# spaceandtimefdn/blitzar

Hardware: AMD Instinct MI355X
Metric: MSM throughput (scalar-point ops/sec) (higher is better)
Workload: dtype u32; 1 GPU; curve25519_msm_n2^20_252bit; columns_per_gpu=1, rows=1048576, parallelism=columns x1

## Files before the change

### __graft_entry__.py

```python
import os
import subprocess
import sys

ROOT = os.path.dirname(os.path.abspath(__file__))
if ROOT not in sys.path:
    sys.path.insert(0, ROOT)


def build():
    from blitzar_amd import build as bz_build
    bz_build.build()
    hooks_dir = os.path.join(ROOT, "tests", "native", "_build")
    os.makedirs(hooks_dir, exist_ok=True)
    hooks = os.path.join(hooks_dir, "libbz_hooks.so")
    src = os.path.join(ROOT, "tests", "native", "hooks.cpp")
    if not os.path.exists(hooks) or os.path.getmtime(hooks) < os.path.getmtime(src):
        subprocess.run(["g++", "-O2", "-std=c++20", "-fPIC", "-shared", "-I" + ROOT, src, "-o", hooks],
                       check=True)
    src = os.path.join(ROOT, "tests", "native", "tile_digest_check.cc")
    newest = max(os.path.getmtime(src),
                 os.path.getmtime(os.path.join(ROOT, "blitzar_amd", "csrc", "msm", "tile_digest.h")))
    for exe, flags in (("tile_digest_check", ["-O2"]),
                       ("tile_digest_check_san", ["-O1", "-g", "-fsanitize=address,undefined",
                                                  "-fno-sanitize-recover=all"])):
        exe = os.path.join(hooks_dir, exe)
        if not os.path.exists(exe) or os.path.getmtime(exe) < newest:
            subprocess.run(["g++", *flags, "-std=c++20", "-I" + ROOT, src, "-o", exe], check=True)
    src = os.path.join(ROOT, "tests", "native", "batch_normalise_check.cc")
    newest = os.path.getmtime(src)
    for d, _, fs in os.walk(os.path.join(ROOT, "blitzar_amd", "csrc")):
        newest = max([newest] + [os.path.getmtime(os.path.join(d, f)) for f in fs if f.endswith(".h")])
    for exe, flags in (("batch_normalise_check", ["-O2"]),
                       ("batch_normalise_check_san", ["-O1", "-g", "-fsanitize=address,undefined",
                                                      "-fno-sanitize-recover=all"])):
        exe = os.path.join(hooks_dir, exe)
        if not os.path.exists(exe) or os.path.getmtime(exe) < newest:
            subprocess.run(["g++", *flags, "-std=c++20", "-I" + ROOT, src, "-o", exe], check=True)
    pb_dir = os.path.join(ROOT, "tools", "pipeline_bench")
    lib_so = os.path.join(ROOT, "blitzar_amd", "lib", "libblitzar_amd.so")
    os.makedirs(os.path.join(pb_dir, "_build"), exist_ok=True)
    for tool in ("pipeline_bench", "multi_device_check", "hostapi_bench", "caller_table_bench"):
        exe = os.path.join(pb_dir, "_build", tool)
        src = os.path.join(pb_dir, tool + ".cc")
        if (not os.path.exists(exe)
                or os.path.getmtime(exe) < max(os.path.getmtime(src), os.path.getmtime(lib_so))):
            subprocess.run(["/opt/rocm/bin/hipcc", "-O2", "-std=c++17",
                            "-I" + os.path.join(ROOT, "include"), "-I" + pb_dir, src,
                            "-L" + os.path.dirname(lib_so), "-lblitzar_amd",
                            "-Wl,-rpath,$ORIGIN/../../../blitzar_amd/lib", "-o", exe], check=True)
    mc_src = os.path.join(ROOT, "tools", "multi_commitment", "benchmark.cc")
    mc_exe = os.path.join(ROOT, "tools", "multi_commitment", "_build", "multi_commitment")
    os.makedirs(os.path.dirname(mc_exe), exist_ok=True)
    if (not os.path.exists(mc_exe)
            or os.path.getmtime(mc_exe) < max(os.path.getmtime(mc_src), os.path.getmtime(lib_so))):
        subprocess.run(["g++", "-O2", "-std=c++17", "-I" + os.path.join(ROOT, "include"), mc_src,
                        "-L" + os.path.dirname(lib_so), "-lblitzar_amd",
                        "-Wl,-rpath,$ORIGIN/../../../blitzar_amd/lib", "-Wl,-rpath,/opt/rocm/lib",
                        "-o", mc_exe], check=True)
    exe = os.path.join(hooks_dir, "sig_ours")
    src = os.path.join(ROOT, "tests", "native", "boundary", "signatures.cc")
    if (not os.path.exists(exe)
            or os.path.getmtime(exe) < max(os.path.getmtime(src), os.path.getmtime(lib_so))):
        subprocess.run(["g++", "-O1", "-std=c++17", "-I" + os.path.join(ROOT, "include"),
                        '-DBZ_API_HEADER="blitzar_api.h"', src, "-L" + os.path.dirname(lib_so),
                        "-lblitzar_amd", "-Wl,-rpath,$ORIGIN/../../../blitzar_amd/lib",
                        "-Wl,-rpath,/opt/rocm/lib", "-o", exe], check=True)
    mt_dir = os.path.join(ROOT, "tools", "mt19937")
    mt_so = os.path.join(mt_dir, "_build", "libmtstream.so")
    mt_src = os.path.join(mt_dir, "mtstream.cc")
    os.makedirs(os.path.dirname(mt_so), exist_ok=True)
    if not os.path.exists(mt_so) or os.path.getmtime(mt_so) < os.path.getmtime(mt_src):
        subprocess.run(["g++", "-O2", "-std=c++17", "-fPIC", "-shared", "-pthread", mt_src, "-o",
                        mt_so], check=True)
    subprocess.run([sys.executable, os.path.join(ROOT, "oracle", "ref", "build_ref.py")], check=True)
    from tests import device_hooks
    device_hooks.build()
    import blitzar_amd.api as api
    api.load()


def smoke():
    import numpy as np
    from blitzar_amd import api
    from oracle import ref_oracle
    lib = api.load()
    assert lib.bzamd_device_count() > 0, "smoke() needs a GPU"
    api.reset_for_testing()
    assert api.init(api.SXT_GPU_BACKEND, 16) == 0
    rng = np.random.default_rng(0)
    n = 1000
    cols = [(rng.integers(0, 256, (n, 32), dtype=np.uint8), False),
            (rng.integers(0, 256, (n, 4), dtype=np.uint8), True)]
    before = lib.bzamd_kernel_launch_count()
    got = api.compute_pedersen_commitments(0, cols)
    assert lib.bzamd_kernel_launch_count() > before, "no kernels were launched"
    if ref_oracle.available():
        want = ref_oracle.commit(0, cols, ref_oracle.ristretto_generators(n))
        assert np.array_equal(got, want), "HIP MSM disagrees with the reference oracle"
    golden = api.compute_pedersen_commitments(0, [(np.array([2000, 7500, 5000, 1500], np.uint32), False)])
    assert golden[0, :4].tolist() == [4, 105, 58, 131]
    a = rng.integers(0, 256, (5, 32), dtype=np.uint8)
    b = rng.integers(0, 256, (5, 32), dtype=np.uint8)
    t0 = api.transcript_new("smoke")
    l, r, ap, t1 = api.prove_inner_product(t0, 5, 2, a, b)
    if ref_oracle.available():
        wl, wr, wap, wt = ref_oracle.ip_prove(t0, 5, 2, a, b)
        assert np.array_equal(l, wl) and np.array_equal(r, wr) and np.array_equal(ap, wap)
        assert np.array_equal(t1, wt), "inner-product proof disagrees with the reference prover"
    api.reset_for_testing()
    print("smoke ok")


if __name__ == "__main__":
    build()
```

### blitzar_amd/csrc/msm/curve_traits.h

```cpp
#pragma once

#include "blitzar_amd/csrc/curve/ed25519.h"
#include "blitzar_amd/csrc/curve/ed29.h"
#include "blitzar_amd/csrc/curve/ed16_wave.h"
#include "blitzar_amd/csrc/curve/sw29.h"
#include "blitzar_amd/csrc/curve/sw29_coop.h"
#include "blitzar_amd/csrc/curve/sw_wave.h"
#include "blitzar_amd/csrc/curve/weierstrass.h"

namespace bz {

template <int N> struct sw_api_affine {
  u64 X[N];
  u64 Y[N];
  u8 infinity;
};
static_assert(sizeof(sw_api_affine<4>) == 72);
static_assert(sizeof(sw_api_affine<6>) == 104);

struct ed25519_msm {
  static constexpr unsigned curve_id = 0;
  using point = ed29_point;
  using addend = ed29_cached_packed;
  using api_projective = ed_point;
// ... 3 lines not shown
  static constexpr size_t output_size = 32;
  static constexpr size_t projective_size = 160;
  static constexpr int accumulate_waves_per_simd = 3;
  static constexpr int accumulate_launch_waves = 2;
  static constexpr bool has_batched_prepare = false;
  static constexpr double call_table_entry_cost = 1.0;

  BZ_HD static point identity() { return ed29::identity(); }
  BZ_HD static point add(const point& a, const point& b) { return ed29::add(a, b); }
  BZ_HD static point dbl_n(const point& a, int k) { return ed29::dbl_n(a, k); }
  BZ_HD static point neg(const point& a) { return ed29::neg(a); }
  BZ_HD static void accumulate(point& acc, const addend& q, bool negate) {
    acc = ed29::add_cached(acc, ed29::unpack(q), negate);
  }
  using operand = ed29_cached;
  BZ_HD static operand stage(const addend& q) {
    operand o = ed29::unpack(q);
    f29::pin(o.YpX);
    f29::pin(o.YmX);
    f29::pin(o.Z);
    f29::pin(o.T2d);
    return o;
  }
  BZ_HD static void accumulate(point& acc, const operand& q, bool negate) {
    acc = ed29::add_cached(acc, q, negate);
  }
  static constexpr bool has_signed_gather = true;
  BZ_HD static addend gather(const addend* table, u32 row, bool negate) {
    return ed29::gather_signed(table, row, negate);
  }
  BZ_HD static void accumulate_gathered(point& acc, const operand& q, bool negate) {
    acc = ed29::add_cached_presigned(acc, q, negate);
  }
  static constexpr bool first_pinned = true;
  BZ_HD static point first_gathered(const operand& q, bool negate) {
    return ed29::from_cached_presigned(q, negate);
  }
  BZ_HD static addend make_addend(const void* api_generators, u64 i) {
    return ed29::pack(ed29::cached_from_ed(static_cast<const ed_point*>(api_generators)[i]));
  }
  BZ_HD static addend addend_from_api_projective(const void* projective, u64 i) {
    return make_addend(projective, i);
  }
  BZ_HD static void encode(u8* out, const point& p) { ristretto29::encode(out, p); }
  BZ_HD static void store_projective(u8* out, const point& p) {
    *reinterpret_cast<ed_point*>(out) = ed29::to_ed(p);
  }
  BZ_HD static point point_from_api_projective(const void* projective, u64 i) {
    return ed29::from_ed(static_cast<const ed_point*>(projective)[i]);
  }
  BZ_HD static void store_api_generator(u8* out, const point& p) { store_projective(out, p); }
  BZ_HD static point point_from_api_generator(const void* api_generators, u64 i) {
    return point_from_api_projective(api_generators, i);
  }
  static constexpr u32 batch_points_per_lane = 4;
  using batch_fe = fe29;
  BZ_HD static fe29 batch_one() { return f29::one(); }
  BZ_HD static fe29 batch_mul(const fe29& a, const fe29& b) { return f29::mul(a, b); }
  BZ_HD static bool batch_is_zero(const fe29& a) { return f29::is_zero(a); }
  BZ_HD static fe29 batch_z(const point& p, bool& is_identity) {
    is_identity = false;
    return p.Z;
  }
  static constexpr size_t compact_size = 120;
  BZ_HD static void store_compact(u8* out, const point& p, const fe29& zinv, bool) {
    const fe29 x = f29::mul(p.X, zinv), y = f29::mul(p.Y, zinv);
    const fe51 c[3] = {f29::to_fe51(x), f29::to_fe51(y), f29::to_fe51(f29::mul(x, y))};
    u64* o = reinterpret_cast<u64*>(out);
    for (int k = 0; k < 3; ++k)
      for (int i = 0; i < 5; ++i) o[5 * k + i] = c[k].v[i];
  }
#if defined(__HIPCC__)
  __device__ static fe29 batch_wave_invert(const fe29& z) {
    return batch_wave_invert(z, ed16w::wave_scratch());
  }
  __device__ static fe29 batch_wave_invert(const fe29& z, ed16w::scratch* lds) {
    const ed16w::lane_ctx c = ed16w::make_ctx(lds);
    const fe29 t = ed16w::pow22523(c, z);
    return f29::mul(f29::sqn(t, 3), f29::mul(f29::sq(z), z));
  }
#endif
  static constexpr bool has_wave_horner = true;
#if defined(__HIPCC__)
  __device__ static point wave_horner(const point& acc, bool have_acc, point* window_sums,
                                      u32 stride, u32 num_windows, u32 window_bits) {
    const ed16w::lane_ctx c = ed16w::make_ctx(ed16w::wave_scratch());
    for (u32 w = c.lane; w < num_windows; w += 64) {
      point* slot = window_sums + static_cast<size_t>(w) * stride;
      const ed29_cached_packed q = ed29::pack(ed29::to_cached(*slot));
      *reinterpret_cast<ed29_cached_packed*>(slot) = q;
    }
    ed16w::wave_lds_sync();
    u32 state = ed16w::identity(c);
    if (have_acc) state = ed16w::load_point(c, acc);
    for (u32 i = num_windows; i-- > 0;) {
      if (have_acc || i + 1 != num_windows) {
        for (u32 k = 0; k < window_bits; ++k) state = ed16w::dbl(c, state);
      }
      const u32* q = reinterpret_cast<const u32*>(window_sums + static_cast<size_t>(i) * stride);
      state = ed16w::add_cached(c, state, ed16w::load_words(c, q));
    }
    return ed16w::store_point(c, state);
  }
  __device__ static void wave_chain(point* out, u64 stride, const point& g, u32 windows, u32 bits) {
    const ed16w::lane_ctx c = ed16w::make_ctx(ed16w::wave_scratch());
    u32 state = ed16w::load_point(c, g);
#pragma unroll 1
    for (u32 w = 0;; ++w) {
      const point p = ed16w::store_point(c, state);
      if (c.lane == 0) out[static_cast<u64>(w) * stride] = p;
      if (w + 1 >= windows) break;
#pragma unroll 1
      for (u32 k = 0; k < bits; ++k) state = ed16w::dbl(c, state);
    }
  }
  static constexpr bool has_wave_add_multiple = true;
  static constexpr bool reduce_scan_few_columns_only = false;
  __device__ static point wave_add_multiple(const point& v, const point& s, u32 m) {
    __shared__ ed29_cached_packed addend[2];
    const ed16w::lane_ctx c = ed16w::make_ctx(ed16w::wave_scratch());
    if (c.lane < 2) addend[c.lane] = ed29::pack(ed29::to_cached(c.lane == 0 ? s : v));
    ed16w::wave_lds_sync();
    const u32 sq = ed16w::load_words(c, addend[0].w), vq = ed16w::load_words(c, addend[1].w);
    u32 state = ed16w::identity(c);
    for (int bit = 31 - __builtin_clz(m); bit >= 0; --bit) {
      state = ed16w::dbl(c, state);
      if ((m >> bit) & 1) state = ed16w::add_cached(c, state, sq);
    }
    state = ed16w::add_cached(c, state, vq);
    return ed16w::store_point(c, state);
  }
  static constexpr bool has_wave_encode = true;
  static constexpr bool has_coop_add = false;
  __device__ static void wave_encode(u8* out, const point& p) {
    const ed16w::lane_ctx c = ed16w::make_ctx(ed16w::wave_scratch());
    u64 w[4];
    ristretto29::encode_words(w, p, [&c](const fe29& z) { return ed16w::pow22523(c, z); });
    if (c.lane == 0) {
      for (int i = 0; i < 4; ++i)
        for (int j = 0; j < 8; ++j) out[8 * i + j] = static_cast<u8>(w[i] >> (8 * j));
    }
  }
#endif
};

struct ed25519_niels_msm : ed25519_msm {
  using addend = ed29_niels;
  static constexpr int accumulate_launch_waves = accumulate_waves_per_simd;
  BZ_HD static void accumulate(point& acc, const addend& q, bool negate) {
    acc = ed29::add_niels(acc, q, negate);
  }
  BZ_HD static point first(const addend& q, bool negate) { return ed29::from_niels(q, negate); }
  static constexpr bool has_signed_gather = false;
  static constexpr double call_table_entry_cost = 0.88;
  using operand = ed29_niels;
  BZ_HD static operand stage(const addend& q) {
    operand o = q;
    f29::pin(o.YpX);
    f29::pin(o.YmX);
    f29::pin(o.T2d);
    return o;
  }
  BZ_HD static addend make_addend(const void* api_generators, u64 i) {
    return ed29::to_niels(ed29::from_ed(static_cast<const ed_point*>(api_generators)[i]));
  }
  BZ_HD static addend addend_from_api_projective(const void* projective, u64 i) {
    return make_addend(projective, i);
  }
  static constexpr bool has_batched_prepare = true;
  BZ_HD static fe29 batch_load_z(const void* api_generators, u64 i) {
    return f29::from_fe51(static_cast<const ed_point*>(api_generators)[i].Z);
  }
  BZ_HD static void batch_load_xyz(const void* api_generators, u64 i, fe29& big_x, fe29& big_y,
                                   fe29& z) {
    const ed_point& g = static_cast<const ed_point*>(api_generators)[i];
    big_x = f29::from_fe51(g.X);
    big_y = f29::from_fe51(g.Y);
    z = f29::from_fe51(g.Z);
  }
#if defined(__HIPCC__)
  using batch_scratch = ed16w::scratch;
#endif
  BZ_HD static addend batch_make_addend(const void* api_generators, u64 i, const fe29& zinv) {
    const ed_point& g = static_cast<const ed_point*>(api_generators)[i];
    return niels_of(f29::from_fe51(g.X), f29::from_fe51(g.Y), zinv);
  }
  BZ_HD static addend addend_from_point(const point& p, const fe29& zinv, bool) {
    return niels_of(p.X, p.Y, zinv);
  }
  BZ_HD static addend niels_of(const fe29& big_x, const fe29& big_y, const fe29& zinv) {
    const fe29 x = f29::mul(big_x, zinv);
    const fe29 y = f29::mul(big_y, zinv);
    ed29_niels n;
    n.YpX = f29::weak_reduce(f29::add(y, x));
    n.YmX = f29::weak_reduce(f29::sub(y, x));
    n.T2d = f29::mul(f29::mul(x, y), f29::const_2d());
    for (int k = 0; k < 5; ++k) n.pad[k] = 0;
    return n;
  }
};

template <class G29, unsigned CurveId> struct sw_msm_base {
  static constexpr unsigned curve_id = CurveId;
  static constexpr double call_table_entry_cost = 1.0;
  using G64 = typename G29::G64;
  using F64 = typename G64::F;
  static constexpr int N64 = F64::N;
  using point = typename G29::point;
  using addend = typename G29::packed;
  using api_projective = typename G64::point;
  using api_affine = sw_api_affine<N64>;
  static constexpr size_t api_generator_size = sizeof(api_affine);
  static constexpr size_t projective_size = sizeof(api_projective);
  static constexpr int accumulate_waves_per_simd = G29::N <= 9 ? 3 : 2;
  static constexpr int accumulate_launch_waves = accumulate_waves_per_simd;
  static constexpr bool accumulate_pinned = G29::N <= 9;
  static constexpr bool has_batched_prepare = false;
  static constexpr bool has_signed_gather = false;
  static constexpr bool has_wave_encode = false;
  static constexpr bool has_wave_add_multiple = true;
  static constexpr bool reduce_scan_few_columns_only = true;
#if defined(__HIPCC__)
  __device__ static point wave_add_multiple(const point& v, const point& s, u32 m) {
    using W = sww::wave<G29>;
    const typename W::ctx c = W::make_ctx(sww::wave_scratch());
    const u32 sq = W::load_point_value(c, s), vq = W::load_point_value(c, v);
    u32 st = sq;
    for (int bit = 30 - __builtin_clz(m); bit >= 0; --bit) {
      st = W::dbl(c, st);
      if ((m >> bit) & 1) st = W::add(c, st, sq);
    }
    return W::store_point(c, W::add(c, st, vq));
  }
#endif
  static constexpr bool has_wave_horner = true;
#if defined(__HIPCC__)
  __device__ static void wave_chain(point* out, u64 stride, const point& g, u32 windows, u32 bits) {
    using W = sww::wave<G29>;
    const typename W::ctx c = W::make_ctx(sww::wave_scratch());
    u32 st = W::load_point_value(c, g);
#pragma unroll 1
    for (u32 w = 0;; ++w) {
      const point p = W::store_point(c, st);
      if (c.lane == 0) out[static_cast<u64>(w) * stride] = p;
      if (w + 1 >= windows) break;
#pragma unroll 1
      for (u32 k = 0; k < bits; ++k) st = W::dbl(c, st);
    }
  }
  __device__ static point wave_horner(point acc, bool have_acc, point* window_sums,
                                      u32 stride, u32 num_windows, u32 window_bits) {
    return sww::wave<G29>::horner(sww::wave_scratch(), acc, have_acc, window_sums, stride,
                                  num_windows, window_bits);
  }
#endif

  static constexpr bool has_coop_add = true;
#if defined(__HIPCC__)
  __device__ static point add_coop4(const point& a, const point& b, u32 role) {
    return sw29_coop::add_coop4<G29>(a, b, role);
  }
#endif

  using F29 = typename G29::F;
  using batch_fe = typename G29::fe;
  BZ_HD static batch_fe batch_one() { return F29::one(); }
  BZ_HD static batch_fe batch_mul(const batch_fe& a, const batch_fe& b) { return F29::mul(a, b); }
  BZ_HD static batch_fe batch_z(const point& p, bool& is_identity) {
    is_identity = F29::is_zero(p.Z);
    return is_identity ? F29::one() : p.Z;
  }
  BZ_HD static batch_fe batch_wave_invert(const batch_fe& z) { return F29::invert(z); }
  static constexpr size_t compact_size = 16 * N64;
  BZ_HD static void store_compact(u8* out, const point& p, const batch_fe& zinv, bool is_identity) {
    u64* o = reinterpret_cast<u64*>(out);
    if (is_identity) {
      const typename G64::F::fe one = G64::F::one();
      for (int k = 0; k < N64; ++k) {
        o[k] = k == N64 - 1 ? ~u64{0} : 0;
        o[N64 + k] = one.v[k];
      }
      return;
    }
    F29::to_mont64(o, F29::mul(p.X, zinv));
    F29::to_mont64(o + N64, F29::mul(p.Y, zinv));
  }

  BZ_HD static point identity() { return G29::identity(); }
  BZ_HD static point add(const point& a, const point& b) { return G29::add(a, b); }
  BZ_HD static point dbl_n(const point& a, int k) { return G29::dbl_n(a, k); }
  BZ_HD static void accumulate(point& acc, const addend& q, bool negate) {
    if (G29::is_identity_addend(q)) return;
    acc = G29::template add_mixed<accumulate_pinned>(acc, G29::unpack(q), negate);
  }
  struct operand {
    typename G29::affine a;
    u32 nonzero;
  };
  BZ_HD static operand stage(const addend& q) {
    u64 any = 0;
#pragma unroll
    for (int i = 0; i < N64; ++i) any |= q.x[i] | q.y[i];
    operand o{G29::unpack(q), static_cast<u32>(any) | static_cast<u32>(any >> 32)};
    F29::pin(o.a.x);
    F29::pin(o.a.y);
#if defined(__HIP_DEVICE_COMPILE__)
// ... 78 lines not shown
```

### blitzar_amd/csrc/msm/kernels.h

```cpp
#pragma once

#include <utility>

#include "blitzar_amd/csrc/msm/batch_tree.h"
#include "blitzar_amd/csrc/msm/curve_traits.h"
#include "blitzar_amd/csrc/msm/plan.h"
#include "blitzar_amd/csrc/msm/recode.h"
#include "blitzar_amd/csrc/msm/tile_digest.h"

namespace bz {

using i16 = int16_t;
using i32 = int32_t;
template <class D> inline constexpr u32 kDigitsPerVector = 16 / sizeof(D);

constexpr u32 kSortThreads = 1024;
constexpr u32 kReduceHeavyHeads = 16;
constexpr u32 kReduceMaxHeavy = 8;
constexpr u32 kAccumulateThreads = 256;
constexpr u32 kCombineThreads = 256;

template <class C>
__global__ void __launch_bounds__(256)
    k_prepare_addends(typename C::addend* __restrict__ addends, const void* __restrict__ api_generators,
                      u64 n) {
  const u64 i = static_cast<u64>(blockIdx.x) * blockDim.x + threadIdx.x;
  if (i >= n) return;
  addends[i] = C::make_addend(api_generators, i);
}

template <class C, u32 T>
__device__ __forceinline__ void tree_products(typename C::batch_fe* tree, u32 tid) {
  __syncthreads();
  for (u32 s = T / 2; s >= 1; s >>= 1) {
    tree_product_step<C>(tree, s, tid);
    __syncthreads();
  }
}
template <class C, u32 T>
__device__ __forceinline__ void tree_inverses(typename C::batch_fe* tree, u32 tid) {
  __syncthreads();
  for (u32 s = 1; s < T; s <<= 1) {
    tree_inverse_step<C>(tree, s, tid);
    __syncthreads();
  }
}

__device__ __forceinline__ void wave_lds_fence() {
  __builtin_amdgcn_fence(__ATOMIC_RELEASE, "workgroup");
  __builtin_amdgcn_wave_barrier();
  __builtin_amdgcn_fence(__ATOMIC_ACQUIRE, "workgroup");
}
struct caller_table_view {
  tile_digest* tiles;
  tile_digest* rows;
  u64 valid_rows;
  unsigned long long* converted;
};
constexpr u32 kConvertedCounters = 256, kConvertedCounterStride = 16;
template <class C, bool Table = false>
__global__ void __launch_bounds__(256)
    k_prepare_addends_staged(typename C::addend* __restrict__ addends,
                             const void* __restrict__ api_generators, u64 n,
                             caller_table_view table) {
  using addend = typename C::addend;
  constexpr bool Norm = Table && C::has_batched_prepare;
  static_assert(Table || !C::has_batched_prepare, "Z = 1 addends outside a table: the batched kernel");
  constexpr u32 G = static_cast<u32>(C::api_generator_size);
  constexpr u32 A = static_cast<u32>(sizeof(addend));
  static_assert(G % 8 == 0 && A % 16 == 0 && A <= G && (64 * G) % 16 == 0);
  __shared__ __attribute__((aligned(16))) u8 stage[4 * 64 * G];
  const u32 lane = threadIdx.x & 63;
  const u32 wave = Table ? __builtin_amdgcn_readfirstlane(threadIdx.x >> 6) : threadIdx.x >> 6;
  const u64 first = (static_cast<u64>(blockIdx.x) * 4 + wave) * 64;
  if constexpr (!Norm) {
    if (first >= n) return;
  }
  const u32 count = first >= n ? 0 : static_cast<u32>(n - first < 64 ? n - first : 64);
  bool convert = count != 0;
  u8* region = stage + wave * (64 * G);
  const u8* src = static_cast<const u8*>(api_generators) + first * G;
  const u32 in_bytes = count * G;
  const u64 tile = first >> 6;
  tile_digest state{}, stored{};
  bool tile_known = false;
  if constexpr (Table) {
    tile_known = convert && first < table.valid_rows;
    if (tile_known) stored = table.tiles[tile];
    state = digest_lane_begin(lane, count);
  }
  constexpr u32 kRounds = (64 * G / 16 + 63) / 64;
  uint4 words[kRounds];
#pragma unroll
  for (u32 r = 0; r < kRounds; ++r) {
    const u32 off = (r * 64 + lane) * 16;
    if (off + 16 <= in_bytes) words[r] = *reinterpret_cast<const uint4*>(src + off);
  }
#pragma unroll
  for (u32 r = 0; r < kRounds; ++r) {
    const u32 off = (r * 64 + lane) * 16;
    if (off + 16 <= in_bytes) {
      const uint4 v = words[r];
      *reinterpret_cast<uint4*>(region + off) = v;
      if constexpr (Table) {
        state = digest_absorb(state, off >> 4, v.x | static_cast<u64>(v.y) << 32,
                              v.z | static_cast<u64>(v.w) << 32);
      }
    }
  }
  if ((in_bytes & 8) != 0 && lane == 0) {
    const u64 v = *reinterpret_cast<const u64*>(src + in_bytes - 8);
    *reinterpret_cast<u64*>(region + in_bytes - 8) = v;
    if constexpr (Table) state = digest_absorb(state, in_bytes >> 4, v, 0);
  }
  tile_digest whole{}, mine{};
  if constexpr (Table) {
    state = digest_lane_end(state);
    for (int m = 32; m >= 1; m >>= 1) {
      state.a ^= __shfl_xor(state.a, m, 64);
      state.b ^= __shfl_xor(state.b, m, 64);
    }
    whole = digest_finish(state, count);
    if (tile_known && stored.a == whole.a && stored.b == whole.b) {
      if constexpr (!Norm) return;
      convert = false;
    }
  }
  if (convert) wave_lds_fence();
  if (Table && convert) {
    const bool known = lane < count && first + lane < table.valid_rows;
    tile_digest was{};
    if (known) was = table.rows[first + lane];
    bool same = lane >= count;
    if (lane < count) {
      mine = digest_of_row(reinterpret_cast<const u64*>(region + lane * G), G, lane);
      same = known && was.a == mine.a && was.b == mine.b;
    }
    if (__all(same)) {
      if (count == 64 && lane == 0) table.tiles[tile] = whole;
      if constexpr (!Norm) return;
      convert = false;
    }
  }
  addend a;
  if constexpr (Norm) {
    using fe = typename C::batch_fe;
    constexpr u32 T = 256;
    static_assert(sizeof(fe) * 2 * T % 16 == 0 &&
                  sizeof(fe) * 2 * T + sizeof(typename C::batch_scratch) <= sizeof(stage));
    const bool live = convert && lane < count;
    fe big_x, big_y, z;
    if (live) C::batch_load_xyz(region, lane, big_x, big_y, z);
    wave_lds_fence();
    if (lane == 0) *reinterpret_cast<u32*>(region) = convert ? 1u : 0u;
    __syncthreads();
    u32 any = 0;
#pragma unroll
    for (u32 w = 0; w < 4; ++w) any |= *reinterpret_cast<const u32*>(stage + w * (64 * G));
// ... 854 lines not shown
        run_base[b0 + 1] = gstart1 + (c1 != 0 ? atomicAdd(&fill[b0 + 1], c1) : 0);
      }
      lds_barrier();
#pragma unroll
      for (u32 k = 0; k < kLocalSortPerThread; ++k) {
        const bool active = tid + k * kGroupSortThreads < total;
        const u32 b = (mine[k] >> shift) & in_group;
        const u32 pos = wave_aggregated_add(cursor, b, active);
        if (active) staging[pos] = mine[k];
      }
      lds_barrier();
      u32* out = sorted + task.entry_base + group_begin;
      u32* seg = segment_bucket + task.segment_base;
      const u32 seg_log2 = task.segment_log2, seg_mask = (1u << seg_log2) - 1;
      for (u32 i = tid; i < total; i += kGroupSortThreads) {
        const u32 r = staging[i];
        const u32 b = (r >> shift) & in_group;
        const u32 at = run_base[b] + (i - local_start[b]);
        out[at] = ((r & 0x80000000u) | (r & row_mask)) + task.row_base;
        if (((group_begin + at) & seg_mask) == 0) {
          seg[(group_begin + at) >> seg_log2] = (g << s) + b;
        }
      }
      lds_barrier();
    }
  }
}

template <class D>
__global__ void __launch_bounds__(kGroupSortThreads, 8)
    k_task_sort(u32* __restrict__ sorted, u32* __restrict__ segment_bucket,
                u32* __restrict__ bucket_end, const D* __restrict__ digits,
                const task_desc* __restrict__ tasks) {
  __shared__ sort_lds lds;
  u32* cursor = lds.cursor;
  u32* staging = lds.staging;
  u32* wave_sums = lds.wave_sums;
  const task_desc task = tasks[blockIdx.x];
  const u32 buckets = task.num_buckets;
  const u32 rows = static_cast<u32>(task.rows);
  const u32 tid = threadIdx.x, lane = tid & 63, wave = tid >> 6;
  for (u32 b = tid; b < buckets; b += kGroupSortThreads) cursor[b] = 0;
  lds_barrier();
  const D* dig = digits + task.entry_base;
  u32 mine[kLocalSortPerThread];
  u32 rank2[(kLocalSortPerThread + 1) / 2];
#pragma unroll
  for (u32 k = 0; k < kLocalSortPerThread; ++k) {
    const u32 i = tid + k * kGroupSortThreads;
    const int e = i < rows ? static_cast<int>(dig[i]) : 0;
    const u32 mag = e < 0 ? static_cast<u32>(-e) : static_cast<u32>(e);
    mine[k] = e == 0 ? 0u : ((e > 0 ? 0x80000000u : 0u) | ((mag - 1) << 13) | i | 0x40000000u);
    u32 r = 0;
    if (e != 0) r = atomicAdd(&cursor[mag - 1], 1u);
    if ((k & 1) == 0) {
      rank2[k / 2] = r;
    } else {
      rank2[k / 2] |= r << 16;
    }
  }
  lds_barrier();
  const u32 b0 = 2 * tid;
  const u32 c0 = b0 < buckets ? cursor[b0] : 0, c1 = b0 + 1 < buckets ? cursor[b0 + 1] : 0;
  const u32 local = c0 + c1;
  u32 incl = local;
#pragma unroll
  for (u32 off = 1; off < 64; off <<= 1) {
    const u32 up = __shfl_up(incl, off, 64);
    if (lane >= off) incl += up;
  }
  if (lane == 63) wave_sums[wave] = incl;
  lds_barrier();
  u32 start0 = incl - local;
  u32 total = 0;
  for (u32 w = 0; w < kGroupSortThreads / 64; ++w) {
    if (w < wave) start0 += wave_sums[w];
    total += wave_sums[w];
  }
  const u32 start1 = start0 + c0;
  u32* ends = bucket_end + task.bucket_base;
  if (b0 < buckets) {
    cursor[b0] = start0;
    ends[b0] = start0 + c0;
  }
  if (b0 + 1 < buckets) {
    cursor[b0 + 1] = start1;
    ends[b0 + 1] = start1 + c1;
  }
  lds_barrier();
  u32* seg = segment_bucket + task.segment_base;
  const u32 seg_log2 = task.segment_log2, seg_mask = (1u << seg_log2) - 1;
#pragma unroll
  for (u32 k = 0; k < kLocalSortPerThread; ++k) {
    if (mine[k] != 0) {
      const u32 b = (mine[k] >> 13) & 0x3ffu;
      const u32 at = cursor[b] + ((rank2[k / 2] >> (16 * (k & 1))) & 0xffffu);
      staging[at] = (mine[k] & 0x80000000u) | (mine[k] & 0x1fffu);
      if ((at & seg_mask) == 0) seg[at >> seg_log2] = b;
    }
  }
  lds_barrier();
  u32* out = sorted + task.entry_base;
  for (u32 i = tid; i < total; i += kGroupSortThreads) out[i] = staging[i] + task.row_base;
}

static __global__ void __launch_bounds__(kGroupSortThreads, 8)
    k_group_sort_all(u32* __restrict__ sorted, u32* __restrict__ segment_bucket,
                     u32* __restrict__ bucket_end, const u32* __restrict__ records,
                     const u32* __restrict__ group_start, const u32* __restrict__ group_chunk,
                     const task_desc* __restrict__ tasks, u32 num_tasks,
                     u32* __restrict__ bucket_count, u32* __restrict__ bucket_fill,
                     const u32* __restrict__ big_tasks, u32* __restrict__ big_barrier,
                     u32 max_workers) {
  __shared__ sort_lds lds;
  if (blockIdx.y < num_tasks) {
    const task_desc task = tasks[blockIdx.y];
    group_sort_block(blockIdx.x, task, sorted, segment_bucket, bucket_end, records, group_start,
                     group_chunk, lds);
    return;
  }
  const u32 workers = gridDim.x < max_workers ? gridDim.x : max_workers;
  if (blockIdx.x >= workers) return;
  const u32 num_big_tasks = big_tasks[0];
  if (num_big_tasks == 0) return;
  big_hist_body(blockIdx.x, workers, bucket_count, records, group_start, group_chunk, tasks,
                big_tasks, num_big_tasks, lds.cursor);
  __shared__ big_sort_lds big;
  asm volatile("s_waitcnt vmcnt(0)" ::: "memory");
  __syncthreads();
  if (threadIdx.x == 0) {
    __hip_atomic_fetch_add(big_barrier, 1u, __ATOMIC_RELAXED, __HIP_MEMORY_SCOPE_AGENT);
    while (__hip_atomic_load(big_barrier, __ATOMIC_RELAXED, __HIP_MEMORY_SCOPE_AGENT) < workers) {
      __builtin_amdgcn_s_sleep(16);
    }
  }
  __syncthreads();
  big_sort_body(blockIdx.x, workers, sorted, segment_bucket, bucket_end, bucket_count, bucket_fill,
                records, group_start, group_chunk, tasks, big_tasks, num_big_tasks, lds, big);
}

template <class P> __device__ __forceinline__ P wave_shfl_down(const P& v, u32 delta) {
  static_assert(sizeof(P) % 4 == 0);
  P r;
  const u32* src = reinterpret_cast<const u32*>(&v);
  u32* dst = reinterpret_cast<u32*>(&r);
#pragma unroll
  for (u32 i = 0; i < sizeof(P) / 4; ++i) dst[i] = __shfl_down(src[i], delta, 64);
  return r;
}

constexpr int kReducePrio = 3;
constexpr int kHornerPrio = 3;
template <class C>
__global__ void __launch_bounds__(kAccumulateThreads, C::accumulate_launch_waves)
    k_accumulate(typename C::point* __restrict__ bucket_sums, typename C::point* __restrict__ heads,
                 const u32* __restrict__ bucket_end, const u32* __restrict__ segment_bucket,
                 const u32* __restrict__ sorted, const typename C::addend* __restrict__ addends,
                 const task_desc* __restrict__ tasks) {
  const task_desc task = tasks[blockIdx.y];
  const u32* ends = bucket_end + task.bucket_base;
  const u32 total = ends[task.num_buckets - 1];
  const u32 seg = blockIdx.x * kAccumulateThreads + threadIdx.x;
  const u32 seg_entries = 1u << task.segment_log2;
  const u32 lo = seg << task.segment_log2;
  if (lo >= total) return;
  const u32 hi = lo + seg_entries < total ? lo + seg_entries : total;
  u32 b = segment_bucket[task.segment_base + seg];
  u32 b_end = ends[b];
  const u32 b_start = b == 0 ? 0 : ends[b - 1];
  bool owned = b_start == lo;
  const bool whole = !owned && b_end >= lo + seg_entries;
  const u32* idx = sorted + task.entry_base;
  typename C::point* sums = bucket_sums + task.bucket_base;
  typename C::point acc = C::identity();
  const u32 last_bucket = task.num_buckets - 1;
  u32 next_end = ends[b < last_bucket ? b + 1 : last_bucket];
  typename C::point* flush_to = owned ? sums + b : heads + task.segment_base + seg;
  u32 e_cur = *(idx + lo);
  u32 e_next = lo + 1 < hi ? *(idx + lo + 1) : 0;
  auto gather = [&](u32 entry) {
    if constexpr (C::has_signed_gather) {
      return C::gather(addends, entry & 0x7fffffffu, (entry >> 31) != 0);
    } else {
      return addends[entry & 0x7fffffffu];
    }
  };
  typename C::addend staged = gather(e_cur);
  {
    const typename C::operand q = C::stage(staged);
    const bool negate = (e_cur >> 31) != 0;
    const u32 next_entry = lo + 1 < hi ? e_next : e_cur;
    e_cur = e_next;
    staged = gather(next_entry);
    if (lo + 2 < hi) e_next = *(idx + lo + 2);
    if constexpr (C::has_signed_gather) {
      acc = C::first_gathered(q, negate);
    } else {
      acc = C::first(q, negate);
    }
    if constexpr (C::first_pinned) {
      u32* w = reinterpret_cast<u32*>(&acc);
#pragma unroll
      for (u32 k = 0; k < sizeof(acc) / 4; ++k) asm volatile("" : "+v"(w[k]));
    }
  }
  for (u32 i = lo + 1; i < hi; ++i) {
    const typename C::operand q = C::stage(staged);
    const bool negate = (e_cur >> 31) != 0;
    if (i == b_end) {
      *flush_to = acc;
      ++b;
      b_end = next_end;
      while (b_end == i) {
        ++b;
        b_end = ends[b];
      }
      flush_to = sums + b;
      owned = true;
      acc = C::identity();
    }
    next_end = ends[b < last_bucket ? b + 1 : last_bucket];
    const u32 next_entry = i + 1 < hi ? e_next : e_cur;
    e_cur = e_next;
    staged = gather(next_entry);
    if (i + 2 < hi) e_next = *(idx + i + 2);
    if constexpr (C::has_signed_gather) {
      C::accumulate_gathered(acc, q, negate);
    } else {
      C::accumulate(acc, q, negate);
    }
  }
  const unsigned long long whole_mask = __ballot(whole);
  const u32 lane = threadIdx.x & 63;
  bool write_head = !owned;
  if ((whole_mask & (whole_mask >> 1)) != 0) {
    const u32 run = whole ? static_cast<u32>(__ffsll(static_cast<long long>(~(whole_mask >> lane)))) - 1 : 0;
    for (u32 d = 1; d < 64; d <<= 1) {
      const typename C::point other = wave_shfl_down(acc, d);
      if (whole && d < run) acc = C::add(acc, other);
    }
    if (whole && lane != 0 && ((whole_mask >> (lane - 1)) & 1) != 0) write_head = false;
  }
  if (owned || write_head) *flush_to = acc;
}

#define BZ_ACCUMULATE_INSTANCE(KEYWORD, C)                                                         \
  KEYWORD template __global__ void k_accumulate<C>(                                                \
      typename C::point* __restrict__, typename C::point* __restrict__, const u32* __restrict__,   \
      const u32* __restrict__, const u32* __restrict__, const typename C::addend* __restrict__,    \
      const task_desc* __restrict__)

template <class C>
__device__ __forceinline__ typename C::point
load_bucket(const typename C::point* __restrict__ sums, const typename C::point* __restrict__ heads,
            u32 begin, u32 end, u32 b, u32 seg_log2) {
  typename C::point v = sums[b];
  const u32 first = begin >> seg_log2, last = (end - 1) >> seg_log2;
  const u32 after_whole = end >> seg_log2;
  u32 s = first + 1;
  while (s <= last) {
    v = C::add(v, heads[s]);
    if (s < after_whole) {
      const u32 next_wave = (s / 64 + 1) * 64;
      s = next_wave < after_whole ? next_wave : after_whole;
    } else {
      ++s;
    }
  }
  return v;
}

struct bucket_heads {
  u32 s0, k_lo, middle, tail_index, count;
  __device__ __forceinline__ u32 index(u32 j) const {
    return j == 0 ? s0 : (j <= middle ? (k_lo + j - 1) * 64 : tail_index);
  }
};
__device__ __forceinline__ bucket_heads heads_of(u32 begin, u32 end, u32 seg_log2) {
  const u32 first = begin >> seg_log2, last = (end - 1) >> seg_log2;
  const u32 after_whole = end >> seg_log2;
  bucket_heads h;
  h.s0 = first + 1;
  h.k_lo = h.s0 / 64 + 1;
  const u32 k_hi_plus_1 = (after_whole + 63) / 64;
  h.middle = k_hi_plus_1 > h.k_lo ? k_hi_plus_1 - h.k_lo : 0;
  h.tail_index = after_whole;
  const u32 tail = after_whole <= last && after_whole > h.s0 ? 1 : 0;
  h.count = h.s0 > last ? 0 : 1 + h.middle + tail;
  return h;
}

template <class C, bool Scan, u32 T = kReduceThreads>
__global__ void __launch_bounds__(T)
    k_reduce(typename C::point* __restrict__ partials, u32 partial_stride,
             u32* __restrict__ task_total, const typename C::point* __restrict__ bucket_sums,
             const typename C::point* __restrict__ heads, const u32* __restrict__ bucket_end,
             const task_desc* __restrict__ tasks, u32 lane_log2) {
  using point = typename C::point;
  __shared__ point tree[T];
  __builtin_amdgcn_s_setprio(kReducePrio);
  const task_desc task = tasks[blockIdx.y];
  const u32 nb = task.num_buckets;
  const u32 seg_log2 = task.segment_log2;
  const u32 lane_buckets = 1u << lane_log2;
  const u32 block_first = blockIdx.x * (T << lane_log2);
  if (block_first >= nb) return;
  const u32 tid = threadIdx.x;
  const u32* ends = bucket_end + task.bucket_base;
  const u32 total = ends[nb - 1];
  if (blockIdx.x == 0 && tid == 0) task_total[blockIdx.y] = total;
  point* dst = partials + static_cast<u64>(blockIdx.y) * partial_stride + blockIdx.x;
// ... 461 lines not shown
```

Before: 1.207 billion scalar-point ops/s.

## Gather ed25519 addends through LDS via global_load_lds in bucket accumulation

Adds an accumulate path for the ed25519 curve in which each wave loads the 112-byte addend rows of all 64 lanes with coalesced-by-piece global_load_lds instructions into a per-wave shared-memory region. Each lane then reads its own row back from LDS. The next entry's load is issued before the current point addition so the fetch overlaps the arithmetic. It also changes launch bounds to amdgpu_waves_per_eu to pin occupancy. The cost is 28KB of LDS per block, wave-uniform trip counts that leave lanes idle on short segments, and explicit waitcnt handling.

```diff
diff --git a/__graft_entry__.py b/__graft_entry__.py
--- a/__graft_entry__.py
+++ b/__graft_entry__.py
@@ -33,6 +33,15 @@
     for exe, flags in (("batch_normalise_check", ["-O2"]),
                        ("batch_normalise_check_san", ["-O1", "-g", "-fsanitize=address,undefined",
                                                       "-fno-sanitize-recover=all"])):
+        exe = os.path.join(hooks_dir, exe)
+        if not os.path.exists(exe) or os.path.getmtime(exe) < newest:
+            subprocess.run(["g++", *flags, "-std=c++20", "-I" + ROOT, src, "-o", exe], check=True)
+    src = os.path.join(ROOT, "tests", "native", "lds_gather_check.cc")
+    newest = max(os.path.getmtime(src),
+                 os.path.getmtime(os.path.join(ROOT, "blitzar_amd", "csrc", "msm", "lds_gather.h")))
+    for exe, flags in (("lds_gather_check", ["-O2"]),
+                       ("lds_gather_check_san", ["-O1", "-g", "-fsanitize=address,undefined",
+                                                 "-fno-sanitize-recover=all"])):
         exe = os.path.join(hooks_dir, exe)
         if not os.path.exists(exe) or os.path.getmtime(exe) < newest:
             subprocess.run(["g++", *flags, "-std=c++20", "-I" + ROOT, src, "-o", exe], check=True)
diff --git a/blitzar_amd/csrc/msm/curve_traits.h b/blitzar_amd/csrc/msm/curve_traits.h
--- a/blitzar_amd/csrc/msm/curve_traits.h
+++ b/blitzar_amd/csrc/msm/curve_traits.h
@@ -179,6 +179,7 @@
   }
   BZ_HD static point first(const addend& q, bool negate) { return ed29::from_niels(q, negate); }
   static constexpr bool has_signed_gather = false;
+  static constexpr bool has_lds_gather = true;
   static constexpr double call_table_entry_cost = 0.88;
   using operand = ed29_niels;
   BZ_HD static operand stage(const addend& q) {
diff --git a/blitzar_amd/csrc/msm/kernels.h b/blitzar_amd/csrc/msm/kernels.h
--- a/blitzar_amd/csrc/msm/kernels.h
+++ b/blitzar_amd/csrc/msm/kernels.h
@@ -4,6 +4,7 @@
 
 #include "blitzar_amd/csrc/msm/batch_tree.h"
 #include "blitzar_amd/csrc/msm/curve_traits.h"
+#include "blitzar_amd/csrc/msm/lds_gather.h"
 #include "blitzar_amd/csrc/msm/plan.h"
 #include "blitzar_amd/csrc/msm/recode.h"
 #include "blitzar_amd/csrc/msm/tile_digest.h"
@@ -1164,11 +1165,143 @@
 constexpr int kReducePrio = 3;
 constexpr int kHornerPrio = 3;
 template <class C>
-__global__ void __launch_bounds__(kAccumulateThreads, C::accumulate_launch_waves)
+__device__ __forceinline__ void
+accumulate_lds_gather(typename C::point* __restrict__ bucket_sums, typename C::point* __restrict__ heads,
+                      const u32* __restrict__ bucket_end, const u32* __restrict__ segment_bucket,
+                      const u32* __restrict__ sorted, const typename C::addend* __restrict__ addends,
+                      const task_desc* __restrict__ tasks) {
+  namespace lg = lds_gather;
+  static_assert(sizeof(typename C::addend) == 128 && sizeof(typename C::operand) >= lg::kRowBytes);
+  static_assert(!C::has_signed_gather);
+  __shared__ __attribute__((aligned(16))) u8 regions[kAccumulateThreads / 64][lg::kRegionBytes];
+  const task_desc task = tasks[blockIdx.y];
+  const u32* ends = bucket_end + task.bucket_base;
+  const u32 total = ends[task.num_buckets - 1];
+  const u32 lane = threadIdx.x & 63;
+  const u32 seg = blockIdx.x * kAccumulateThreads + threadIdx.x;
+  const u32 seg_entries = 1u << task.segment_log2;
+  const u32 lo = seg << task.segment_log2;
+  const u32 wave_lo = __builtin_amdgcn_readfirstlane(lo);
+  if (wave_lo >= total) return;
+  const u32 trips = lg::wave_trips(wave_lo, seg_entries, total);
+  const bool has = lo < total;
+  const u32 hi = lg::lane_hi(lo, seg_entries, total);
+  u32 b = has ? segment_bucket[task.segment_base + seg] : 0;
+  u32 b_end = ends[b];
+  const u32 b_start = b == 0 ? 0 : ends[b - 1];
+  bool owned = has && b_start == lo;
+  const bool whole = has && !owned && b_end >= lo + seg_entries;
+  const u32* idx = sorted + task.entry_base;
+  typename C::point* sums = bucket_sums + task.bucket_base;
+  typename C::point acc = C::identity();
+  const u32 last_bucket = task.num_buckets - 1;
+  u32 next_end = ends[b < last_bucket ? b + 1 : last_bucket];
+  typename C::point* flush_to = owned ? sums + b : heads + task.segment_base + seg;
+
+  u8* region = regions[threadIdx.x >> 6];
+  auto issue = [&](u32 entry) {
+    const u32 row = entry & 0x7fffffffu;
+    u32 rows[lg::kPieces];
+#pragma unroll
+    for (u32 i = 0; i < lg::kPieces; ++i) {
+      rows[i] = static_cast<u32>(
+          __shfl(static_cast<int>(row), static_cast<int>(lg::piece_of(i, lane).source_lane), 64));
+    }
+#pragma unroll
+    for (u32 i = 0; i < lg::kPieces; ++i) {
+      const u8* src = reinterpret_cast<const u8*>(addends) +
+                      static_cast<u64>(rows[i]) * sizeof(typename C::addend) +
+                      lg::piece_of(i, lane).chunk * lg::kPieceBytes;
+      __builtin_amdgcn_global_load_lds(
+          (const __attribute__((address_space(1))) void*)src,
+          (__attribute__((address_space(3))) void*)(region + lg::instruction_base(i)),
+          lg::kPieceBytes, 0, 0);
+    }
+  };
+  constexpr int kWaitVm0 = 0x0f70, kWaitLgkm0 = 0xc07f;
+  auto land = [&]() {
+    __builtin_amdgcn_s_waitcnt(kWaitVm0);
+    asm volatile("" ::: "memory");
+    typename C::operand q;
+    u32* w = reinterpret_cast<u32*>(&q);
+#pragma unroll
+    for (u32 j = 0; j < lg::kPieces; ++j) {
+      const uint4 v = *reinterpret_cast<const uint4*>(region + lg::read_offset(lane, j));
+      w[4 * j] = v.x, w[4 * j + 1] = v.y, w[4 * j + 2] = v.z, w[4 * j + 3] = v.w;
+    }
+    __builtin_amdgcn_s_waitcnt(kWaitLgkm0);
+    asm volatile("" ::: "memory");
+    return C::stage(q);
+  };
+
+  u32 e_cur = has ? *(idx + lo) : 0;
+  const u32 wave_entry = static_cast<u32>(__shfl(static_cast<int>(e_cur), 0, 64));
+  e_cur = lg::valid_entry(has, e_cur, wave_entry);
+  issue(e_cur);
+  u32 e_next = lo + 1 < hi ? *(idx + lo + 1) : 0;
+  {
+    const typename C::operand q = land();
+    const bool negate = (e_cur >> 31) != 0;
+    e_cur = lg::valid_entry(lo + 1 < hi, e_next, e_cur);
+    if (trips > 1) issue(e_cur);
+    if (lo + 2 < hi) e_next = *(idx + lo + 2);
+    acc = C::first(q, negate);
+    if constexpr (C::first_pinned) {
+      u32* w = reinterpret_cast<u32*>(&acc);
+#pragma unroll
+      for (u32 k = 0; k < sizeof(acc) / 4; ++k) asm volatile("" : "+v"(w[k]));
+    }
+  }
+  for (u32 k = 1; k < trips; ++k) {
+    const u32 i = lo + k;
+    const bool act = i < hi;
+    const typename C::operand q = land();
+    const bool negate = (e_cur >> 31) != 0;
+    e_cur = lg::valid_entry(i + 1 < hi, e_next, e_cur);
+    if (act && i == b_end) {
+      *flush_to = acc;
+      ++b;
+      b_end = next_end;
+      while (b_end == i) {
+        ++b;
+        b_end = ends[b];
+      }
+      flush_to = sums + b;
+      owned = true;
+      acc = C::identity();
+    }
+    next_end = ends[b < last_bucket ? b + 1 : last_bucket];
+    if (k + 1 < trips) issue(e_cur);
+    if (i + 2 < hi) e_next = *(idx + i + 2);
+    if (act) C::accumulate(acc, q, negate);
+  }
+  const unsigned long long whole_mask = __ballot(whole);
+  bool write_head = has && !owned;
+  if ((whole_mask & (whole_mask >> 1)) != 0) {
+    const u32 run = whole ? static_cast<u32>(__ffsll(static_cast<long long>(~(whole_mask >> lane)))) - 1 : 0;
+    for (u32 d = 1; d < 64; d <<= 1) {
+      const typename C::point other = wave_shfl_down(acc, d);
+      if (whole && d < run) acc = C::add(acc, other);
+    }
+    if (whole && lane != 0 && ((whole_mask >> (lane - 1)) & 1) != 0) write_head = false;
+  }
+  if (owned || write_head) *flush_to = acc;
+}
+
+template <class C> inline constexpr bool kHasLdsGather = requires { requires C::has_lds_gather; };
+
+template <class C>
+__global__ void __launch_bounds__(kAccumulateThreads)
+    __attribute__((amdgpu_waves_per_eu(C::accumulate_launch_waves,
+                                       kHasLdsGather<C> ? C::accumulate_launch_waves : 0)))
     k_accumulate(typename C::point* __restrict__ bucket_sums, typename C::point* __restrict__ heads,
                  const u32* __restrict__ bucket_end, const u32* __restrict__ segment_bucket,
                  const u32* __restrict__ sorted, const typename C::addend* __restrict__ addends,
                  const task_desc* __restrict__ tasks) {
+  if constexpr (kHasLdsGather<C>) {
+    accumulate_lds_gather<C>(bucket_sums, heads, bucket_end, segment_bucket, sorted, addends, tasks);
+    return;
+  }
   const task_desc task = tasks[blockIdx.y];
   const u32* ends = bucket_end + task.bucket_base;
   const u32 total = ends[task.num_buckets - 1];
diff --git a/blitzar_amd/csrc/msm/lds_gather.h b/blitzar_amd/csrc/msm/lds_gather.h
--- /dev/null
+++ b/blitzar_amd/csrc/msm/lds_gather.h
@@ -0,0 +1,35 @@
+#pragma once
+
+#include "blitzar_amd/csrc/base/macros.h"
+
+namespace bz::lds_gather {
+constexpr u32 kLanes = 64;
+constexpr u32 kPieceBytes = 16;
+constexpr u32 kPieces = 7;
+constexpr u32 kRowBytes = kPieces * kPieceBytes;
+constexpr u32 kInstructionBytes = kLanes * kPieceBytes;
+constexpr u32 kRegionBytes = kPieces * kInstructionBytes;
+static_assert(kRegionBytes == kLanes * kRowBytes && kRegionBytes == 7168);
+
+struct piece {
+  u32 source_lane;
+  u32 chunk;
+};
+BZ_HD constexpr piece piece_of(u32 i, u32 lane) {
+  const u32 c = kLanes * i + lane;
+  return {c / kPieces, c % kPieces};
+}
+BZ_HD constexpr u32 instruction_base(u32 i) { return kInstructionBytes * i; }
+BZ_HD constexpr u32 landing_offset(u32 i, u32 lane) { return instruction_base(i) + kPieceBytes * lane; }
+BZ_HD constexpr u32 read_offset(u32 lane, u32 j) { return kRowBytes * lane + kPieceBytes * j; }
+
+BZ_HD constexpr u32 lane_hi(u32 lo, u32 seg_entries, u32 total) {
+  return lo >= total ? lo : lo + seg_entries < total ? lo + seg_entries : total;
+}
+BZ_HD constexpr u32 wave_trips(u32 wave_lo, u32 seg_entries, u32 total) {
+  return seg_entries < total - wave_lo ? seg_entries : total - wave_lo;
+}
+BZ_HD constexpr u32 valid_entry(bool has_next, u32 next_entry, u32 current_entry) {
+  return has_next ? next_entry : current_entry;
+}
+}
```

Measured after the change: 1.247 billion scalar-point ops/s (median of 6 runs). +3.3%, better.
